# jl6017/AutoURDF

Measured on AMD Instinct MI355X. Metric: registered frames/sec (N=4096 pts, K=20 clusters), higher is better.
Workload: dtype f32

## Files before the change

autourdf_amd/csrc/train_engine.hip:

```cpp
#include <cfloat>
#include <chrono>
#include <cmath>
#include <cstdlib>
#include <cstring>
#include <type_traits>
#include <vector>
#include "creg_common.h"
#include "nn_l1.h"

namespace creg {

struct Dims {
    int rot, K, KP, IN, H, HA, HB, H2, OA, OB, NP, NT, epochs;
    float slope;
    int oW1, ob1, oW2, ob2, oW3A, ob3A, oW3B, ob3B, NPAR;
    int nbx, nby;
    int nyb;
    int npb;
    int ppl;
    int nbt, nbp;
    int rows;
};

constexpr int PS_MAXB = 512;
// ... 535 lines not shown
                const unsigned idx = (unsigned)(key[sl] & 0xFFFFull);
                unsigned u = 0xFFFFFFFFu;
                if (idx != 0xFFFFu) {
                    const float4 p = W.pts4[idx];
                    u = ordered_bits(axis == 0 ? p.x : axis == 1 ? p.y : p.z);
                }
                key[sl] = ((unsigned long long)u << 16) | idx;
            }
            __syncthreads();
            bitonic_segments(key, npow, 64 >> sub, tid, 512);
        }
    for (int sl = tid; sl < ns; sl += 512) {
        const unsigned idx = (unsigned)(key[sl] & 0xFFFFull);
        float4 o = make_float4(0.f, 0.f, 0.f, __int_as_float(0x7fffffff));
        if (idx != 0xFFFFu) { const float4 p = W.pts4[idx]; o = make_float4(p.x, p.y, p.z, __int_as_float((int)idx)); }
        W.psl4[(size_t)first * BS + sl] = o;
    }
}

struct EngineEpi {
    int* sgn_x; int4* cnt4; float* lossp_x; float* lossp_y;
    size_t bstride;
    const int* stopped;
    __device__ __forceinline__ void shift(int z) {
        const size_t b = (size_t)z * bstride;
        sgn_x = (int*)((char*)sgn_x + b); cnt4 = (int4*)((char*)cnt4 + b);
        lossp_x = (float*)((char*)lossp_x + b); lossp_y = (float*)((char*)lossp_y + b);
        stopped = (const int*)((const char*)stopped + b);
    }
    __device__ __forceinline__ void operator()(int dir, int q, int idx, float d, float qx, float qy, float qz,
                                               float tx, float ty, float tz, float& acc) const {
        if (dir == 0) {
            sgn_x[q] = (qx > tx ? 1 : 0) | (qy > ty ? 2 : 0) | (qz > tz ? 4 : 0);
        } else {
            atomicAdd(&cnt4[idx].x, (qx > tx) ? -1 : 1);
            atomicAdd(&cnt4[idx].y, (qy > ty) ? -1 : 1);
            atomicAdd(&cnt4[idx].z, (qz > tz) ? -1 : 1);
        }
        acc += d;
    }
    __device__ __forceinline__ void finish(int dir, int blk, float s, float*) const { (dir == 0 ? lossp_x : lossp_y)[blk] = s; }
};

template <bool P1, int PPL, int NBT, int NBP>
__global__ __launch_bounds__(NN_BLOCK) void k_nn_plan(const float* A, int na, const float* B, int nb, int blocksA,
                                                      int blocksB, EngineEpi epi, NnBlocks yb, NnBlocks pb, size_t zstride) {
    asm volatile("" :: "s"(A), "s"(na), "s"(B), "s"(nb), "s"(blocksA), "s"(blocksB), "s"(epi.sgn_x), "s"(epi.cnt4), "s"(epi.lossp_x), "s"(epi.lossp_y),
                 "s"(epi.bstride), "s"(epi.stopped), "s"(yb.ts4), "s"(yb.tbox), "s"(yb.nblk), "s"(pb.ts4), "s"(pb.tbox), "s"(pb.nblk_dev), "s"(zstride));
    const int nz = gridDim.x / (blocksA + blocksB);
    int i = blockIdx.x, z, bx;
    if (i < blocksB * nz) { z = i / blocksB; bx = blocksA + (i - z * blocksB); }
    else { i -= blocksB * nz; z = i / blocksA; bx = i - z * blocksA; }
    const size_t zb = z * zstride;
    A = (const float*)((const char*)A + zb);
    B = (const float*)((const char*)B + zb);
    yb.ts4 = (const float4*)((const char*)yb.ts4 + zb);
    yb.tbox = (const float*)((const char*)yb.tbox + zb);
    epi.shift(z);
    if (bx < blocksA) nn_l1_block_pruned<NBT, PPL, EngineEpi, true, false>(A, na, 4, yb, 0, epi, bx, epi.stopped, B, 4);
    else if constexpr (P1) {
        pb.ts4 = (const float4*)((const char*)pb.ts4 + zb);
        pb.tbox = (const float*)((const char*)pb.tbox + zb);
        pb.nblk_dev = (const int*)((const char*)pb.nblk_dev + zb);
        nn_l1_block_pruned<NBP, PPL, EngineEpi, true, true>(B, nb, 4, pb, 1, epi, bx - blocksA, epi.stopped, A, 4);
    } else nn_l1_block<4, int, EngineEpi>(A, na, 4, B, nb, 4, nullptr, nullptr, nullptr, nullptr, blocksA, epi, bx);
}

template <int NBT, int NBP>
__global__ __launch_bounds__(NN_ROWS_BLOCK) void k_nn_rows(const float* A, const float* B, int blocksA, int blocksB, EngineEpi epi, NnBlocks yb, NnBlocks pb,
                                                      size_t zstride) {
    asm volatile("" :: "s"(A), "s"(B), "s"(blocksA), "s"(blocksB), "s"(epi.sgn_x), "s"(epi.cnt4), "s"(epi.lossp_x), "s"(epi.lossp_y),
                 "s"(epi.bstride), "s"(epi.stopped), "s"(yb.ts4), "s"(yb.tbox), "s"(yb.nblk), "s"(pb.ts4), "s"(pb.tbox), "s"(pb.nblk_dev), "s"(zstride));
    const int nz = gridDim.x / (blocksA + blocksB);
    int i = blockIdx.x, z, bx;
    if (i < blocksB * nz) { z = i / blocksB; bx = blocksA + (i - z * blocksB); }
    else { i -= blocksB * nz; z = i / blocksA; bx = i - z * blocksA; }
    const size_t zb = z * zstride;
    A = (const float*)((const char*)A + zb);
    B = (const float*)((const char*)B + zb);
    yb.ts4 = (const float4*)((const char*)yb.ts4 + zb);
    yb.tbox = (const float*)((const char*)yb.tbox + zb);
    pb.ts4 = (const float4*)((const char*)pb.ts4 + zb);
    pb.tbox = (const float*)((const char*)pb.tbox + zb);
    pb.nblk_dev = (const int*)((const char*)pb.nblk_dev + zb);
    epi.shift(z);
    if (bx < blocksA) nn_l1_rows<NBT, EngineEpi, false, true>(pb.ts4, 0, pb.nblk_dev, pb.nblk, yb, 0, epi, bx, epi.stopped, B, epi.lossp_x);
    else nn_l1_rows<NBP, EngineEpi, true, false>(yb.ts4, yb.nblk, nullptr, yb.nblk, pb, 1, epi, bx - blocksA, epi.stopped, A, epi.lossp_y);
}

__device__ __forceinline__ TrainState advance_state(const TrainState& S, float loss, const Hyper& hy, double bc1, float bc2_sqrt) {
    TrainState N = S;
    const bool improved = loss < S.min_loss;
    N.last_loss = loss;
    N.epochs_run = S.epochs_run + 1;
    const int count = improved ? 0 : S.count + 1;
    N.min_loss = improved ? loss : S.min_loss;
    N.best_epoch = improved ? S.epochs_run : S.best_epoch;
    N.count = count;
    N.stopped = (!improved && count > hy.stop) ? 1 : S.stopped;
    if (!N.stopped) {
        N.step = S.step + 1;
        N.step_size = (float)(S.lr / bc1);
        N.bc2_sqrt = bc2_sqrt;
        const double cur = (double)loss;
        if (cur < S.sched_best * (1.0 - 1e-4)) { N.sched_best = cur; N.sched_bad = 0; }
        else N.sched_bad = S.sched_bad + 1;
        if (N.sched_bad > hy.patience) {
            const double nl = fmax(S.lr * (double)hy.factor, 0.0);
            if (S.lr - nl > 1e-8) N.lr = nl;
            N.sched_bad = 0;
        }
    }
    return N;
}

constexpr int GC_QMAX = 3;
__device__ __forceinline__ void gradc_role(const Dims& D, const Ws& W, int epoch, int nbx, int nby, int k) {
    __shared__ float red[4][14];
    __shared__ float s_loss;
    __shared__ float s_go[16];
    const int tid = threadIdx.x, lane = tid & 63, wv = tid >> 6;
    const TrainState S = W.state[epoch & 1];
    const int b0 = W.off[k], e0 = W.off[k + 1];
    const Hyper hy = *W.hyper;
    float a = tid < nbx ? W.lossp_x[tid] : 0.f, b = tid < nby ? W.lossp_y[tid] : 0.f;
    const float m2v = W.m2[16 * k + (tid & 15)];
    float sv[16];
#pragma unroll
    for (int i = 0; i < 16; ++i) sv[i] = W.head_save[16 * k + i];
    const float* h2cur = (epoch & 1) ? W.h2[1] : W.h2[0];
    float w3v[GC_QMAX][8], h2v[GC_QMAX];
#pragma unroll
    for (int q = 0; q < GC_QMAX; ++q) {
        const int o = min(q * 256 + tid, D.H2 - 1);
        const bool isA = o < D.HA;
        const float* Pc = (epoch & 1) ? W.P1 : W.P;
        const float* wb = isA ? Pc + D.oW3A + o : Pc + D.oW3B + (o - D.HA);
        const int stride = isA ? D.HA : D.HB, nj = isA ? D.OA : D.OB;
#pragma unroll
        for (int j = 0; j < 8; ++j) w3v[q][j] = wb[(size_t)min(j, nj - 1) * stride];
        h2v[q] = h2cur[(size_t)k * D.H2 + o];
    }
    asm volatile("" :: "v"(a), "v"(b), "v"(m2v), "v"(sv[0]), "v"(sv[1]), "v"(sv[2]), "v"(sv[3]), "v"(sv[4]), "v"(sv[5]), "v"(sv[6]), "v"(sv[7]),
                 "v"(sv[8]), "v"(sv[9]), "v"(sv[10]), "v"(sv[11]), "v"(sv[12]), "v"(sv[13]), "v"(sv[14]), "v"(sv[15]), "v"(b0), "v"(e0), "v"(hy.lr));
#pragma unroll
    for (int q = 0; q < GC_QMAX; ++q)
        asm volatile("" :: "v"(h2v[q]), "v"(w3v[q][0]), "v"(w3v[q][1]), "v"(w3v[q][2]), "v"(w3v[q][3]), "v"(w3v[q][4]), "v"(w3v[q][5]), "v"(w3v[q][6]),
                     "v"(w3v[q][7]));
    if (S.stopped) {
        if (k == 0 && tid == 0) {
            TrainState E = S; E.stopped = 1;
            W.state[(epoch + 1) & 1] = E;
        }
        return;
    }
    const int n_first = min(b0 + tid, D.NP - 1);
    const float4 p_first = W.pts4[n_first];
    const int4 c_first = W.cnt4[n_first];
    const int s_first = W.sgn_x[n_first];
    const float4 pr_first = W.pred4[n_first];
    for (int i = tid + 256; i < nbx; i += 256) a += W.lossp_x[i];
    for (int i = tid + 256; i < nby; i += 256) b += W.lossp_y[i];
    a = wave_sum_fast(a); b = wave_sum_fast(b);
    if (lane == 0) { red[wv][0] = a; red[wv][1] = b; }
    __syncthreads();
    if (tid == 0) {
        const float sa = ((red[0][0] + red[1][0]) + red[2][0]) + red[3][0];
        const float sb = ((red[0][1] + red[1][1]) + red[2][1]) + red[3][1];
        s_loss = sa / (float)D.NP + sb / (float)D.NT;
    }
    __syncthreads();
    const float loss = s_loss;
    TrainState N = advance_state(S, loss, hy, S.next_bc1, S.next_bc2s);
    const bool improved = loss < S.min_loss;
    if (improved) {
        for (int n = b0 + tid; n < e0; n += 256) {
            const float4 p = (n == b0 + tid) ? pr_first : W.pred4[n];
            W.best_pred[3 * (size_t)n] = p.x; W.best_pred[3 * (size_t)n + 1] = p.y; W.best_pred[3 * (size_t)n + 2] = p.z;
        }
        if (tid < 16) W.best_m[16 * k + tid] = m2v;
    }
    if (k == 0 && tid == 0) {
        N.next_bc1 = W.bc1[min(N.step + 1, D.epochs)];
        N.next_bc2s = W.bc2s[min(N.step + 1, D.epochs)];
        W.state[(epoch + 1) & 1] = N;
        W.loss_hist[S.epochs_run] = loss;
        W.lr_hist[S.epochs_run] = (float)S.lr;
        W.result[0] = N.min_loss; W.result[1] = (float)N.epochs_run; W.result[2] = (float)N.lr; W.result[3] = (float)N.best_epoch;
    }
    if (N.stopped) return;
    const float gx = 1.0f / (float)D.NP, gy = 1.0f / (float)D.NT;
    float acc[12];
#pragma unroll
    for (int i = 0; i < 12; ++i) acc[i] = 0.f;
    for (int n = b0 + tid; n < e0; n += 256) {
        const bool first = n == b0 + tid;
        const float4 p = first ? p_first : W.pts4[n];
        const int4 c = first ? c_first : W.cnt4[n];
        const int sb = first ? s_first : W.sgn_x[n];
        const float g[3] = {((sb & 1) ? gx : -gx) + gy * (float)c.x, ((sb & 2) ? gx : -gx) + gy * (float)c.y,
                            ((sb & 4) ? gx : -gx) + gy * (float)c.z};
#pragma unroll
        for (int q = 0; q < 3; ++q) {
            acc[4 * q] = fmaf(g[q], p.x, acc[4 * q]); acc[4 * q + 1] = fmaf(g[q], p.y, acc[4 * q + 1]);
            acc[4 * q + 2] = fmaf(g[q], p.z, acc[4 * q + 2]); acc[4 * q + 3] += g[q];
        }
    }
    __syncthreads();
#pragma unroll
    for (int i = 0; i < 12; ++i) { const float r = wave_sum_fast(acc[i]); if (lane == 0) red[wv][i] = r; }
    __syncthreads();
    if (tid == 0) {
        float G12[12];
        for (int i = 0; i < 12; ++i) G12[i] = ((red[0][i] + red[1][i]) + red[2][i]) + red[3][i];
        for (int i = 0; i < 16; ++i) W.gm2[16 * k + i] = i < 12 ? G12[i] : 0.f;
        const float G[9] = {G12[0], G12[1], G12[2], G12[4], G12[5], G12[6], G12[8], G12[9], G12[10]};
        const float gt[3] = {G12[3], G12[7], G12[11]};
        float go[16];
        for (int i = 0; i < 16; ++i) go[i] = 0.f;
        if (D.rot == ROT_6D) {
            go[0] = gt[0]; go[1] = gt[1]; go[2] = gt[2];
            rot6d_to_matrix_vjp(sv, G, go + 4);
        } else if (D.rot == ROT_RPY) {
            go[0] = gt[0]; go[1] = gt[1]; go[2] = gt[2];
            float ge[3];
            euler_xyz_to_matrix_vjp(sv, G, ge);
            for (int i = 0; i < 3; ++i) go[4 + i] = ge[i] * (1.f - sv[4 + i] * sv[4 + i]);
        } else if (D.rot == ROT_Q) {
            go[0] = gt[0]; go[1] = gt[1]; go[2] = gt[2];
            float gu[4];
            quat_to_matrix_vjp(sv, G, gu);
            const float nrm = sv[4];
            if (nrm > 1e-12f) {
                const float dot = sv[0] * gu[0] + sv[1] * gu[1] + sv[2] * gu[2] + sv[3] * gu[3];
#pragma unroll
                for (int i = 0; i < 4; ++i) go[4 + i] = (gu[i] - sv[i] * dot) / nrm;
            } else {
#pragma unroll
                for (int i = 0; i < 4; ++i) go[4 + i] = gu[i] / 1e-12f;
            }
        } else {
            float gdq[8];
            dq_to_se3_vjp(sv, G, gt, gdq);
            for (int i = 0; i < 8; ++i) go[4 + i] = gdq[i];
        }
        for (int i = 0; i < 12; ++i) { W.g_out[16 * k + i] = go[i]; s_go[i] = go[i]; }
    }
    __syncthreads();
#pragma unroll
    for (int q = 0; q < GC_QMAX; ++q) {
        const int o = q * 256 + tid;
        if (o < D.H2) {
            const bool isA = o < D.HA;
            const int nj = isA ? D.OA : D.OB, gofs = isA ? 0 : 4;
            float sum = 0.f;
#pragma unroll
            for (int j = 0; j < 8; ++j) if (j < nj) sum = fmaf(s_go[gofs + j], w3v[q][j], sum);
            W.g_h2[(size_t)k * D.H2 + o] = sum * act_grad(h2v[q], D.slope);
        }
    }
}

__global__ __launch_bounds__(256) void k_gradc(Dims D, Ws W0, int epoch, int nbx, int nby, size_t bstride) {
    asm volatile("" :: "s"(W0.P), "s"(W0.P1), "s"(W0.h2[0]), "s"(W0.h2[1]), "s"(W0.head_save), "s"(W0.m2), "s"(W0.gm2), "s"(W0.pts4), "s"(W0.pred4),
                 "s"(W0.sgn_x), "s"(W0.cnt4), "s"(W0.lossp_x), "s"(W0.lossp_y), "s"(W0.g_out), "s"(W0.g_h2), "s"(W0.state), "s"(W0.bc1), "s"(W0.bc2s),
                 "s"(W0.best_m), "s"(W0.best_pred), "s"(W0.loss_hist), "s"(W0.lr_hist), "s"(W0.result), "s"(W0.off), "s"(W0.hyper),
                 "s"(D.rot), "s"(D.K), "s"(D.H2), "s"(D.HA), "s"(D.HB), "s"(D.OA), "s"(D.OB), "s"(D.NP), "s"(D.NT), "s"(D.epochs), "s"(D.slope),
                 "s"(D.oW3A), "s"(D.oW3B), "s"(epoch), "s"(nbx), "s"(nby), "s"(bstride));
    const Ws W = ws_shift(W0, blockIdx.z * bstride);
    gradc_role(D, W, epoch, nbx, nby, blockIdx.x);
}

__device__ __forceinline__ float adam_value(float p, float& mm, float& vv, float g, float step_size, float bc2_sqrt) {
    const float b1w = (float)(1.0 - 0.9), b2 = 0.999f, b2w = (float)(1.0 - 0.999);
    mm = mm + b1w * (g - mm);
    vv = vv * b2 + (b2w * g) * g;
    const float denom = sqrtf(vv) / bc2_sqrt + 1e-8f;
    return p + (-step_size * mm) / denom;
}

#ifdef CREG_BD_STAMPS
struct BdStamps {
    unsigned long long first[256], endB[256], endD[256], startB[256], startD[256];
    unsigned long long phase[2][8], blocks[2];
    int armed;
};
__device__ BdStamps g_bd_st;
#define BD_T0 unsigned long long bd_t[8]; int bd_n = 0; if (threadIdx.x == 0) bd_t[bd_n++] = bd_entry;
#define BD_T  if (threadIdx.x == 0) bd_t[bd_n++] = wall_clock64();
#define BD_TEND(role, epoch) do { asm volatile("s_waitcnt vmcnt(0)" ::: "memory"); if (threadIdx.x == 0) { bd_t[bd_n++] = wall_clock64(); \
    if (g_bd_st.armed) { const int sl_ = (epoch) & 255; atomicMin(&g_bd_st.first[sl_], bd_t[0]); \
        atomicMin(role ? &g_bd_st.startD[sl_] : &g_bd_st.startB[sl_], bd_t[0]); atomicMax(role ? &g_bd_st.endD[sl_] : &g_bd_st.endB[sl_], bd_t[bd_n - 1]); \
        for (int k_ = 1; k_ < bd_n; ++k_) atomicAdd(&g_bd_st.phase[role][k_ - 1], bd_t[k_] - bd_t[k_ - 1]); atomicAdd(&g_bd_st.blocks[role], 1ull); } } } while (0)
#else
#define BD_T0
#define BD_T
#define BD_TEND(role, epoch)
#endif
constexpr int BD_THREADS = 512;
constexpr int B2_THREADS = BD_THREADS;
constexpr int B2_WAVES = B2_THREADS / 64;
constexpr int B2_CB = 16;
constexpr int B2_RB = 32;
__host__ __device__ inline int b2_smem_floats(int K, int IN, int H2) {
    return B2_WAVES * B2_RB * B2_CB + K * IN + 2 * K * B2_CB + H2 * B2_CB;
}
__device__ __forceinline__ float row_sum16(float v) {
    CREG_DPP_STEP(v, 0xB1, 0xF);
    CREG_DPP_STEP(v, 0x4E, 0xF);
    CREG_DPP_STEP(v, 0x141, 0xF);
    CREG_DPP_STEP(v, 0x140, 0xF);
    return v;
}

template <int KW, bool X>
__device__ __forceinline__ void bwd2_role(const Dims& D, const Ws& W, int epoch, int blk, float* sh, unsigned long long bd_entry) {
    constexpr int NS = KW / 4;
    constexpr bool V4 = KW % 16 == 0;
    constexpr int NA = V4 ? NS / 4 : NS;
    float* red = sh;
    float* encs = red + B2_WAVES * B2_RB * B2_CB;
    float* gxs = encs + D.K * D.IN;
    float* xt = gxs + D.K * B2_CB;
    float* w2s = xt + D.K * B2_CB;
    const int tid = threadIdx.x, lane = tid & 63, wv = tid >> 6, lj = lane & 15, kk = lane >> 4;
    __builtin_amdgcn_s_waitcnt(0x0F70);
    const int c0 = blk * B2_CB, par = epoch & 1;
    const float* x1cur = par ? W.x1[1] : W.x1[0];
    float* x1next = par ? W.x1[0] : W.x1[1];
    const float* Pc = par ? W.P1 : W.P;
    float* Pn = par ? W.P : W.P1;
    BD_T0
    {
        const float* src = Pc + D.oW2 + (size_t)(wv * KW + (lane >> 2)) * D.H + c0 + 4 * (lane & 3);
        float* dst = w2s + wv * KW * B2_CB;
#pragma unroll
        for (int i = 0; i < KW; i += 16)
            if (i + (lane >> 2) < KW)
                __builtin_amdgcn_global_load_lds((const __attribute__((address_space(1))) void*)(src + (size_t)i * D.H),
                                                 (__attribute__((address_space(3))) void*)(dst + i * B2_CB), 16, 0, 0);
    }
    const float* gbase = W.g_h2 + wv * KW + (V4 ? 4 * kk : kk);
    auto load_a = [&](int row, float* dst) {
        const float* g = gbase + (size_t)min(row, D.K - 1) * D.H2;
#pragma unroll
        for (int q = 0; q < NA; ++q) {
            if constexpr (V4) { const float4 v = *(const float4*)(g + 16 * q); dst[4 * q] = v.x; dst[4 * q + 1] = v.y; dst[4 * q + 2] = v.z; dst[4 * q + 3] = v.w; }
            else dst[q] = g[4 * q];
        }
    };
    float a0[NS], a1[NS];
    const bool two0 = D.K > 16;
    load_a(lj, a0);
    if (two0) load_a(16 + lj, a1);
    const int half = tid >> 8, t2 = tid & 255, row = t2 >> 4, i4 = t2 & 15, hu = c0 + row;
    const bool ain = 4 * i4 < D.IN;
    const int ei = min(4 * i4, D.IN - 4);
    const size_t wi = (size_t)D.oW1 + (size_t)hu * D.IN + ei;
    float4 pw = *(const float4*)(Pc + wi), pm = *(const float4*)(W.AM + wi), pv = *(const float4*)(W.AV + wi);
    const bool ain2 = X && 64 + 4 * i4 < D.IN;
    const int ei2 = min(64 + 4 * i4, D.IN - 4);
    const size_t wi2 = (size_t)D.oW1 + (size_t)hu * D.IN + ei2;
    float4 pw2, pm2, pv2;
    if constexpr (X) { pw2 = *(const float4*)(Pc + wi2); pm2 = *(const float4*)(W.AM + wi2); pv2 = *(const float4*)(W.AV + wi2); }
    float pb = Pc[D.ob1 + hu], mb = W.AM[D.ob1 + hu], vb = W.AV[D.ob1 + hu];
    float xv0 = x1cur[(size_t)min(tid >> 4, D.K - 1) * D.H + c0 + (tid & 15)];
    {
        const int n = D.K * D.IN / 4;
        constexpr int NPC = 8;
#pragma unroll
        for (int c = 0; c < NPC; ++c) {
            const int i = c * B2_THREADS + tid;
            if (i < n)
                __builtin_amdgcn_global_load_lds((const __attribute__((address_space(1))) void*)((const float4*)W.enc + i),
                                                 (__attribute__((address_space(3))) void*)((float4*)encs + c * B2_THREADS + (tid & ~63)), 16, 0, 0);
        }
    }
    __builtin_amdgcn_sched_barrier(0);
    const TrainState S = W.state[(epoch + 1) & 1];
    const bool live = !S.stopped;
    __builtin_amdgcn_sched_barrier(0);
    BD_T
    stage_wait();
    float wb[NS];
#pragma unroll
    for (int s = 0; s < NS; ++s) {
        const int o = V4 ? 16 * (s >> 2) + 4 * kk + (s & 3) : 4 * s + kk;
        wb[s] = w2s[(wv * KW + o) * B2_CB + lj];
    }
    for (int r0 = 0; r0 < D.K; r0 += B2_RB) {
        const int nr = min(B2_RB, D.K - r0);
        const bool two = nr > 16;
        float xv = xv0;
        if (r0) {
            load_a(r0 + lj, a0);
            if (two) load_a(r0 + 16 + lj, a1);
            xv = x1cur[(size_t)min(r0 + (tid >> 4), D.K - 1) * D.H + c0 + (tid & 15)];
        }
        f32x4 acc0 = {0.f, 0.f, 0.f, 0.f}, acc1 = {0.f, 0.f, 0.f, 0.f};
        if (two) {
#pragma unroll
            for (int s = 0; s < NS; ++s) {
                acc0 = __builtin_amdgcn_mfma_f32_16x16x4f32(a0[s], wb[s], acc0, 0, 0, 0);
                acc1 = __builtin_amdgcn_mfma_f32_16x16x4f32(a1[s], wb[s], acc1, 0, 0, 0);
            }
        } else {
#pragma unroll
            for (int s = 0; s < NS; ++s) acc0 = __builtin_amdgcn_mfma_f32_16x16x4f32(a0[s], wb[s], acc0, 0, 0, 0);
        }
        if (r0) __syncthreads();
        {
            float* o = red + (wv * B2_RB + 4 * kk) * B2_CB + lj;
#pragma unroll
            for (int v = 0; v < 4; ++v) { o[v * B2_CB] = acc0[v]; if (two) o[(16 + v) * B2_CB] = acc1[v]; }
        }
        stage_wait();
        __syncthreads();
        if (r0 == 0) { BD_T }
        if (!live) return;
        if (tid < nr * B2_CB) {
            float sum = red[tid];
#pragma unroll
            for (int w2 = 1; w2 < B2_WAVES; ++w2) sum += red[w2 * B2_RB * B2_CB + tid];
            gxs[r0 * B2_CB + tid] = sum * act_grad(xv, D.slope);
        }
    }
    __syncthreads();
    BD_T
    float4 ag = make_float4(0.f, 0.f, 0.f, 0.f), ag2 = make_float4(0.f, 0.f, 0.f, 0.f);
    float gsum = 0.f;
    for (int r = 0; r < D.K; ++r) {
        const float g = gxs[r * B2_CB + row];
        const float4 e = *(const float4*)(encs + r * D.IN + ei);
        ag.x = fmaf(g, e.x, ag.x); ag.y = fmaf(g, e.y, ag.y); ag.z = fmaf(g, e.z, ag.z); ag.w = fmaf(g, e.w, ag.w);
        if constexpr (X) {
            const float4 e2 = *(const float4*)(encs + r * D.IN + ei2);
            ag2.x = fmaf(g, e2.x, ag2.x); ag2.y = fmaf(g, e2.y, ag2.y); ag2.z = fmaf(g, e2.z, ag2.z); ag2.w = fmaf(g, e2.w, ag2.w);
        }
        gsum += g;
    }
    float4 nw;
    nw.x = adam_value(pw.x, pm.x, pv.x, ag.x, S.step_size, S.bc2_sqrt);
    nw.y = adam_value(pw.y, pm.y, pv.y, ag.y, S.step_size, S.bc2_sqrt);
    nw.z = adam_value(pw.z, pm.z, pv.z, ag.z, S.step_size, S.bc2_sqrt);
    nw.w = adam_value(pw.w, pm.w, pv.w, ag.w, S.step_size, S.bc2_sqrt);
    float4 nw2 = make_float4(0.f, 0.f, 0.f, 0.f);
    if constexpr (X) {
        nw2.x = adam_value(pw2.x, pm2.x, pv2.x, ag2.x, S.step_size, S.bc2_sqrt);
        nw2.y = adam_value(pw2.y, pm2.y, pv2.y, ag2.y, S.step_size, S.bc2_sqrt);
        nw2.z = adam_value(pw2.z, pm2.z, pv2.z, ag2.z, S.step_size, S.bc2_sqrt);
        nw2.w = adam_value(pw2.w, pm2.w, pv2.w, ag2.w, S.step_size, S.bc2_sqrt);
    }
    pb = adam_value(pb, mb, vb, gsum, S.step_size, S.bc2_sqrt);
    if (live && half == 0) {
        if (ain) { st4_wt(Pn, wi, nw); st4_wt(W.AM, wi, pm); st4_wt(W.AV, wi, pv); }
        if constexpr (X) if (ain2) { st4_wt(Pn, wi2, nw2); st4_wt(W.AM, wi2, pm2); st4_wt(W.AV, wi2, pv2); }
        if (i4 == 0) { Pn[D.ob1 + hu] = pb; W.AM[D.ob1 + hu] = mb; W.AV[D.ob1 + hu] = vb; }
    }
    BD_T
    for (int r = half; r < D.K; r += 2) {
        const float4 e = *(const float4*)(encs + r * D.IN + ei);
        float v = ain ? fmaf(nw.w, e.w, fmaf(nw.z, e.z, fmaf(nw.y, e.y, nw.x * e.x))) : 0.f;
        if constexpr (X) {
            const float4 e2 = *(const float4*)(encs + r * D.IN + ei2);
            if (ain2) v = fmaf(nw2.w, e2.w, fmaf(nw2.z, e2.z, fmaf(nw2.y, e2.y, fmaf(nw2.x, e2.x, v))));
        }
        v = row_sum16(v) + pb;
        if (i4 == 0) xt[r * B2_CB + row] = act_f(v, D.slope);
    }
    __syncthreads();
    if (live)
        for (int t = tid; t < D.K * (B2_CB / 2); t += B2_THREADS) {
            const int r = t >> 3, c2 = 2 * (t & 7);
            *(nn_f2*)(x1next + (size_t)r * D.H + c0 + c2) = nn_f2{xt[r * B2_CB + c2], xt[r * B2_CB + c2 + 1]};
        }
    BD_TEND(0, epoch);
}


constexpr int DW_UNITS = 16;
constexpr int DW_TILES = 4;
constexpr int DW_KC = 5;
__host__ __device__ inline int dw_blocks(const Dims& D) { return D.H2 / DW_UNITS + 2; }

__device__ __forceinline__ void dw_role(const Dims& D, const Ws& W, int epoch, int blk, unsigned long long bd_entry) {
    const int lane = threadIdx.x & 63, wv = threadIdx.x >> 6, lj = lane & 15, q = lane >> 4;
    __builtin_amdgcn_s_waitcnt(0x0F70);
    const int par = epoch & 1;
    const float* Pc = par ? W.P1 : W.P;
    float* Pn = par ? W.P : W.P1;
    const float* x1cur = par ? W.x1[1] : W.x1[0];
    const float* h2cur = par ? W.h2[1] : W.h2[0];
    asm volatile("" : "+s"(x1cur), "+s"(h2cur));
    const int nb2 = D.H2 / DW_UNITS;
    int u0, nu, n_in, oW, ob, astride, gstride;
    const float *amat, *gmat;
    if (blk < nb2) { u0 = blk * DW_UNITS; nu = DW_UNITS; n_in = D.H; oW = D.oW2 + u0 * D.H; ob = D.ob2 + u0; amat = x1cur; astride = D.H; gmat = W.g_h2 + u0; gstride = D.H2; }
    else if (blk == nb2) { u0 = 0; nu = D.OA; n_in = D.HA; oW = D.oW3A; ob = D.ob3A; amat = h2cur; astride = D.H2; gmat = W.g_out; gstride = 16; }
    else { u0 = 0; nu = D.OB; n_in = D.HB; oW = D.oW3B; ob = D.ob3B; amat = h2cur + D.HA; astride = D.H2; gmat = W.g_out + 4; gstride = 16; }
    if (nu == 0) return;
    if (64 * wv >= n_in) return;
    BD_T0
    const int unit = min(lj, nu - 1);
    const bool ulive = lj < nu;
    const int i0 = 64 * wv;
    const int po = (oW + unit * n_in + i0 + 4 * q) * 4;
    const __amdgpu_buffer_rsrc_t rP = buf_rsrc(Pc, D.NPAR * 4), rM = buf_rsrc(W.AM, D.NPAR * 4), rV = buf_rsrc(W.AV, D.NPAR * 4);
    f32x4 acc[DW_TILES];
#pragma unroll
    for (int t = 0; t < DW_TILES; ++t) acc[t] = f32x4{0.f, 0.f, 0.f, 0.f};
    float gb = 0.f;
    const __amdgpu_buffer_rsrc_t rA = buf_rsrc(amat, (D.KP * astride - (int)(amat - (blk < nb2 ? x1cur : h2cur))) * 4);
    const __amdgpu_buffer_rsrc_t rG = buf_rsrc(gmat, (D.KP * gstride - (blk < nb2 ? u0 : (blk == nb2 ? 0 : 4))) * 4);
    const int aoff = (q * astride + i0 + 16 * (lj & 3) + 4 * (lj >> 2)) * 4, goff = (q * gstride + unit) * 4;
    float bop[DW_KC];
    float4 aop[DW_KC];
    auto load_ops = [&](int s0) {
#pragma unroll
        for (int s = 0; s < DW_KC; ++s) {
            const int r4 = 4 * (s0 + s);
            bop[s] = __uint_as_float(__builtin_amdgcn_raw_buffer_load_b32(rG, goff, r4 * gstride * 4, 0));
            aop[s] = ld_buf4(rA, aoff, r4 * astride * 4);
        }
    };
    auto mfma_ops = [&]() {
#pragma unroll
        for (int s = 0; s < DW_KC; ++s) {
            acc[0] = __builtin_amdgcn_mfma_f32_16x16x4f32(aop[s].x, bop[s], acc[0], 0, 0, 0);
            acc[1] = __builtin_amdgcn_mfma_f32_16x16x4f32(aop[s].y, bop[s], acc[1], 0, 0, 0);
            acc[2] = __builtin_amdgcn_mfma_f32_16x16x4f32(aop[s].z, bop[s], acc[2], 0, 0, 0);
            acc[3] = __builtin_amdgcn_mfma_f32_16x16x4f32(aop[s].w, bop[s], acc[3], 0, 0, 0);
        }
#pragma unroll
        for (int s = 0; s < DW_KC; ++s) gb += bop[s];
    };
    load_ops(0);
    __builtin_amdgcn_sched_barrier(0);
    const TrainState S = W.state[(epoch + 1) & 1];
    float pb = Pc[ob + unit], mb = W.AM[ob + unit], vb = W.AV[ob + unit];
    __builtin_amdgcn_sched_barrier(0);
    float4 pw[DW_TILES], pm[DW_TILES], pv[DW_TILES];
    bool vl[DW_TILES];
#pragma unroll
    for (int v = 0; v < DW_TILES; ++v) {
        vl[v] = ulive && i0 + 16 * v + 4 * q < n_in;
        pw[v] = ld_buf4(rP, po + 64 * v, 0); pm[v] = ld_buf4(rM, po + 64 * v, 0); pv[v] = ld_buf4(rV, po + 64 * v, 0);
        __builtin_amdgcn_sched_barrier(0);
    }
    BD_T
    mfma_ops();
    for (int s0 = DW_KC; 4 * s0 < D.KP; s0 += DW_KC) {
        load_ops(s0);
        __builtin_amdgcn_sched_barrier(0);
        mfma_ops();
    }
    BD_T
    if (S.stopped) return;
#pragma unroll
    for (int v = 0; v < DW_TILES; ++v) {
        float4 nw;
        nw.x = adam_value(pw[v].x, pm[v].x, pv[v].x, acc[0][v], S.step_size, S.bc2_sqrt);
        nw.y = adam_value(pw[v].y, pm[v].y, pv[v].y, acc[1][v], S.step_size, S.bc2_sqrt);
        nw.z = adam_value(pw[v].z, pm[v].z, pv[v].z, acc[2][v], S.step_size, S.bc2_sqrt);
        nw.w = adam_value(pw[v].w, pm[v].w, pv[v].w, acc[3][v], S.step_size, S.bc2_sqrt);
        if (vl[v]) { const int e = po / 4 + 16 * v; st4_wt(Pn, e, nw); st4_wt(W.AM, e, pm[v]); st4_wt(W.AV, e, pv[v]); }
    }
    if (wv == 0) {
        float sum = gb;
        sum += __shfl_xor(gb, 16, 64);
        sum += __shfl_xor(sum, 32, 64);
        pb = adam_value(pb, mb, vb, sum, S.step_size, S.bc2_sqrt);
        if (q == 0 && ulive) { Pn[ob + unit] = pb; W.AM[ob + unit] = mb; W.AV[ob + unit] = vb; }
    }
    BD_TEND(1, epoch);
}

template <int NC, int KW, bool X = false>
__global__ __launch_bounds__(BD_THREADS, 4) void k_bd(Dims D, Ws W0, int epoch, size_t bstride, int nz) {
    extern __shared__ __attribute__((aligned(16))) char smem[];
#ifdef CREG_BD_STAMPS
    const unsigned long long bd_entry = wall_clock64();
#else
    const unsigned long long bd_entry = 0;
#endif
#ifndef CREG_BD_NO_TOUCH
    asm volatile("" :: "s"(W0.P), "s"(W0.P1), "s"(W0.AM), "s"(W0.AV), "s"(W0.enc), "s"(W0.x1[0]), "s"(W0.x1[1]), "s"(W0.h2[0]), "s"(W0.h2[1]),
                 "s"(W0.g_out), "s"(W0.g_h2), "s"(W0.state), "s"(D.K), "s"(D.KP), "s"(D.IN), "s"(D.H), "s"(D.H2), "s"(D.HA), "s"(D.HB), "s"(D.OA),
                 "s"(D.OB), "s"(D.oW1), "s"(D.ob1), "s"(D.oW2), "s"(D.ob2), "s"(D.oW3A), "s"(D.ob3A), "s"(D.oW3B), "s"(D.ob3B), "s"(D.NPAR),
                 "s"(D.slope), "s"(epoch), "s"(bstride), "s"(nz));
#endif
    const int nB = D.H / B2_CB, nD = dw_blocks(D);
    int i = blockIdx.x;
    const bool roleB = i < nB * nz;
    if (!roleB) i -= nB * nz;
    const int n = roleB ? nB : nD, z = i / n, blk = i - z * n;
    const Ws W = ws_shift(W0, (size_t)z * bstride);
#ifdef CREG_BD_ONLY
    if ((CREG_BD_ONLY == 1) != roleB) return;
#endif
    if (roleB) bwd2_role<KW, X>(D, W, epoch, blk, (float*)smem, bd_entry);
    else dw_role(D, W, epoch, blk, bd_entry);
}

__global__ __launch_bounds__(256) void k_params_home(Dims D, Ws W0, size_t bstride, int sidx, int step0) {
    const Ws W = ws_shift(W0, blockIdx.z * bstride);
    if (((W.state[sidx].step - step0) & 1) == 0) return;
    for (int i = blockIdx.x * 256 + threadIdx.x; i < D.NPAR; i += gridDim.x * 256) W.P[i] = W.P1[i];
}

struct ResumeState { double lr, sched_best; int step, epochs_run, sched_bad, count, best_epoch, stopped; float min_loss; };
__global__ void k_set_state(Dims D, Ws W, ResumeState rs) {
    if (threadIdx.x || blockIdx.x) return;
    TrainState s = W.state[0];
    s.lr = rs.lr; s.sched_best = rs.sched_best; s.sched_bad = rs.sched_bad; s.count = rs.count; s.stopped = rs.stopped; s.step = rs.step;
    s.min_loss = rs.min_loss; s.epochs_run = rs.epochs_run; s.best_epoch = rs.best_epoch;
    s.next_bc1 = W.bc1[min(rs.step + 1, D.epochs)]; s.next_bc2s = W.bc2s[min(rs.step + 1, D.epochs)];
    W.state[0] = s; W.state[1] = s;
    W.result[0] = s.min_loss; W.result[1] = (float)s.epochs_run; W.result[2] = (float)s.lr; W.result[3] = (float)s.best_epoch;
}
__global__ void k_get_state(Ws W, int sidx, double* out) {
    if (threadIdx.x || blockIdx.x) return;
    const TrainState s = W.state[sidx];
    out[0] = s.step; out[1] = s.epochs_run; out[2] = s.lr; out[3] = s.sched_best; out[4] = s.sched_bad; out[5] = s.count;
    out[6] = (double)s.min_loss; out[7] = s.best_epoch; out[8] = s.stopped; out[9] = (double)s.last_loss; out[10] = 0.0; out[11] = 0.0;
}

struct Plan {
    creg_train_shape shape;
    Dims D;
    Ws W;
    char* base;
    size_t bytes;
    hipGraphExec_t gexec;
    bool graph_ready;
    int graph_epochs;
    int B;
    int nz;
    size_t bstride;
    int smem_bd;
    int branches;
    bool chain_streams;
    hipStream_t cst[8];
    hipGraphExec_t cexec[8];
    hipEvent_t cfork, cjoin[8];
    hipStream_t cal_stream;
    bool cal_done;
    int probe_us;
    bool target_blocks_valid;
};

static bool make_dims(const creg_train_shape* s, Dims* D) {
    if (!s || s->rot < 0 || s->rot > 3 || s->k < 1 || s->k > 256 || (s->hidden != 64 && s->hidden != 128 && s->hidden != 256 && s->hidden != 512) || s->epochs < 1 || s->n_pred < 1 || s->n_tgt < 1 || s->n_pred >= (1ll << 31) ||
        s->n_tgt >= (1ll << 31))
        return false;
    memset(D, 0, sizeof(*D));
    D->rot = s->rot; D->K = s->k; D->KP = (s->k + 19) / 20 * 20; D->H = s->hidden; D->NP = (int)s->n_pred; D->NT = (int)s->n_tgt; D->epochs = s->epochs;
    if (s->rot == ROT_Q) { D->IN = 56; D->HA = D->H / 2; D->HB = D->H; D->OA = 3; D->OB = 4; D->slope = 0.01f; }
    else if (s->rot == ROT_DQ) { D->IN = 64; D->HA = 0; D->HB = D->H; D->OA = 0; D->OB = 8; D->slope = 0.f; }
    else if (s->rot == ROT_6D) { D->IN = 72; D->HA = D->H / 2; D->HB = D->H; D->OA = 3; D->OB = 6; D->slope = 0.01f; }
    else { D->IN = 48; D->HA = D->H / 2; D->HB = D->H; D->OA = 3; D->OB = 3; D->slope = 0.01f; }
    if (D->K * D->IN / 4 > 8 * 512) return false;
    D->H2 = D->HA + D->HB;
    if (sizeof(float) * b2_smem_floats(D->K, D->IN, D->H2) > 160 * 1024) return false;
    int o = 0;
    D->oW1 = o; o += D->H * D->IN; D->ob1 = o; o += D->H;
    D->oW2 = o; o += D->H2 * D->H; D->ob2 = o; o += D->H2;
    D->oW3A = o; o += D->OA * D->HA; D->ob3A = o; o += D->OA;
    D->oW3B = o; o += D->OB * D->HB; D->ob3B = o; o += D->OB;
    D->NPAR = o;
    if (D->H2 % 32 || D->H % B2_CB || D->H2 > 256 * GC_QMAX) return false;
    const NnGrid g = nn_grid(D->NP, D->NT, true, true, 4);
    D->nbx = g.blocksA; D->nby = g.blocksB;
    const bool rows_fit = D->NT <= 16384 && D->NP < 65535 && (D->NP + 63) / 64 + D->K <= PS_MAXB && g.qw == 4;
    const char* rows_env = getenv("CREG_NN_ROWS");
    const bool rows_pays = D->NT > 64 * 64;
    D->rows = s->nn_search == 0 && rows_fit && (rows_env ? rows_env[0] == '1' : rows_pays);
    D->ppl = (D->rows || D->NT <= 64 * 64) ? 1 : 4;
    const int BS = 64 * D->ppl;
    D->nyb = (s->nn_search != 1 && D->NT <= 4 * YS_CHUNK && g.qw == 4) ? (D->NT + BS - 1) / BS : 0;
    D->npb = (D->nyb && D->NP < 65535 && (D->NP + BS - 1) / BS + D->K <= PS_MAXB) ? (D->NP + BS - 1) / BS + D->K : 0;
    const int nt = (D->nyb + 63) / 64, np = (D->npb + 63) / 64;
    D->nbt = nt <= 1 ? 1 : (nt <= 2 ? 2 : 4);
    D->nbp = np <= 2 ? 2 : (np <= 3 ? 3 : (np <= 4 ? 4 : (np <= 5 ? 5 : (np <= 6 ? 6 : 8))));
    if (D->rows) { D->nbx = 4 * D->npb; D->nby = 4 * D->nyb; }
    return true;
}

static size_t carve(const Dims& D, char* base, Ws* W) {
    size_t o = 0;
    auto take = [&](size_t bytes) -> char* { char* r = base ? base + o : nullptr; o = align_up(o + bytes, 256); return r; };
    const size_t f = sizeof(float);
    Ws w;
    w.P = (float*)take(f * D.NPAR); w.P1 = (float*)take(f * D.NPAR); w.AM = (float*)take(f * D.NPAR); w.AV = (float*)take(f * D.NPAR);
    w.pose_in = (float*)take(f * POSE_IN * D.K); w.enc = (float*)take(f * D.K * D.IN);
    w.x1[0] = (float*)take(f * D.KP * D.H); w.x1[1] = (float*)take(f * D.KP * D.H);
    w.h2[0] = (float*)take(f * D.KP * D.H2); w.h2[1] = (float*)take(f * D.KP * D.H2); w.head_save = (float*)take(f * 16 * D.K);
    w.m2 = (float*)take(f * 16 * D.K); w.gm2 = (float*)take(f * 16 * D.K);
    w.pts4 = (float4*)take(sizeof(float4) * D.NP); w.y4 = (float4*)take(sizeof(float4) * D.NT);
    w.pred4 = (float4*)take(sizeof(float4) * D.NP);
    const size_t bs = 64 * (size_t)D.ppl;
    w.ys4 = (float4*)take(sizeof(float4) * bs * (D.nyb ? D.nyb : 1)); w.ybox = (float*)take(f * 6 * 64 * D.nbt);
    w.psl4 = (float4*)take(sizeof(float4) * bs * (D.npb ? D.npb : 1)); w.ps4 = (float4*)take(sizeof(float4) * bs * (D.npb ? D.npb : 1));
    w.pbox = (float*)take(f * 6 * 64 * D.nbp); w.sb = (int*)take(sizeof(int) * (D.K + 1));
    w.sgn_x = (int*)take(sizeof(int) * D.NP);
    w.cnt4 = (int4*)take(sizeof(int4) * D.NP);
    w.lossp_x = (float*)take(f * D.nbx); w.lossp_y = (float*)take(f * D.nby);
    w.g_out = (float*)take(f * 16 * D.KP); w.g_h2 = (float*)take(f * D.KP * D.H2);
    w.state = (TrainState*)take(sizeof(TrainState) * 2);
    w.bc1 = (double*)take(sizeof(double) * (D.epochs + 1)); w.bc2s = (float*)take(f * (D.epochs + 1));
    w.best_m = (float*)take(f * 16 * D.K); w.best_pred = (float*)take(f * 3 * D.NP);
    w.loss_hist = (float*)take(f * D.epochs); w.lr_hist = (float*)take(f * D.epochs); w.result = (float*)take(f * 4);
    w.off = (int*)take(sizeof(int) * (D.K + 1)); w.hyper = (Hyper*)take(sizeof(Hyper));
    w.ysum = (unsigned long long*)take(sizeof(unsigned long long) * 4);
    if (W) *W = w;
    return o;
}

template <typename F>
static void by_nc(int H, F f) {
    switch (H / 64) {
        case 1: f(std::integral_constant<int, 1>{}); break;
        case 2: f(std::integral_constant<int, 2>{}); break;
        case 4: f(std::integral_constant<int, 4>{}); break;
        default: f(std::integral_constant<int, 8>{}); break;
    }
}
static void launch_l2(Plan* P, int par, hipStream_t s) {
    const Dims& D = P->D; const Ws& W = P->W;
    by_nc(D.H, [&](auto nc) {
        hipLaunchKernelGGL((k_l2<decltype(nc)::value>), dim3(D.H2 / 16, 1, P->nz), dim3(L2_THREADS), 0, s, D, W, par, P->bstride); });
}
static void launch_head(Plan* P, int par, hipStream_t s) {
    const Dims& D = P->D; const Ws& W = P->W;
    by_nc(D.H, [&](auto nc) {
        if (D.OA + D.OB > 8) hipLaunchKernelGGL((k_head<decltype(nc)::value, true>), dim3(D.K, 1, P->nz), dim3(512), 0, s, D, W, par, P->bstride);
        else hipLaunchKernelGGL((k_head<decltype(nc)::value>), dim3(D.K, 1, P->nz), dim3(512), 0, s, D, W, par, P->bstride);
    });
}
template <typename F>
static void by_bd(const Dims& D, F f) {
    by_nc(D.H, [&](auto nc) {
        constexpr int NC = decltype(nc)::value;
        if (D.IN > 64) f(k_bd<NC, 12 * NC, true>);
        else if (D.HA) f(k_bd<NC, 12 * NC>);
        else f(k_bd<NC, 8 * NC>);
    });
}
static void launch_bd(Plan* P, int epoch, hipStream_t s) {
    const Dims& D = P->D; const Ws& W = P->W;
    const int per = D.H / B2_CB + dw_blocks(D);
    by_bd(D, [&](auto kern) { hipLaunchKernelGGL(kern, dim3(per * P->nz), dim3(BD_THREADS), P->smem_bd, s, D, W, epoch, P->bstride, P->nz); });
}
static void launch_nn(const Dims& D, const Ws& W, size_t bstride, int nz, hipStream_t s, int par = 0) {
    const EngineEpi epi{W.sgn_x, W.cnt4, W.lossp_x, W.lossp_y, bstride, &W.state[par].stopped};
    if (D.rows) {
        const NnBlocks yb{W.ys4, W.ybox, D.nyb, nullptr}, pb{W.ps4, W.pbox, D.npb, W.sb + D.K};
        const int blocksA = cdiv(64 * D.npb, NN_ROW_SLOTS), blocksB = cdiv(64 * D.nyb, NN_ROW_SLOTS);
        const dim3 grid((blocksA + blocksB) * nz);
        auto go = [&](auto kern) {
            hipLaunchKernelGGL(kern, grid, dim3(NN_ROWS_BLOCK), 0, s, (const float*)W.pred4, (const float*)W.y4, blocksA, blocksB, epi, yb, pb, bstride);
        };
        auto pick_p = [&](auto nbt) {
            constexpr int NBT = decltype(nbt)::value;
            switch (D.nbp) {
                case 2: go(k_nn_rows<NBT, 2>); break;
                case 3: go(k_nn_rows<NBT, 3>); break;
                case 4: go(k_nn_rows<NBT, 4>); break;
                case 5: go(k_nn_rows<NBT, 5>); break;
                case 6: go(k_nn_rows<NBT, 6>); break;
                default: go(k_nn_rows<NBT, 8>); break;
            }
        };
        switch (D.nbt) {
            case 1: pick_p(std::integral_constant<int, 1>{}); break;
            case 2: pick_p(std::integral_constant<int, 2>{}); break;
            default: pick_p(std::integral_constant<int, 4>{}); break;
        }
    } else if (D.nyb) {
// ... 651 lines not shown
```

Baseline: 164.8.

## Split W1 Adam update to one half-block and batch forward row reductions

```diff
diff --git a/autourdf_amd/csrc/train_engine.hip b/autourdf_amd/csrc/train_engine.hip
--- a/autourdf_amd/csrc/train_engine.hip
+++ b/autourdf_amd/csrc/train_engine.hip
@@ -861,8 +861,9 @@
 constexpr int B2_WAVES = B2_THREADS / 64;
 constexpr int B2_CB = 16;
 constexpr int B2_RB = 32;
+constexpr int B2_NR = 5;
 __host__ __device__ inline int b2_smem_floats(int K, int IN, int H2) {
-    return B2_WAVES * B2_RB * B2_CB + K * IN + 2 * K * B2_CB + H2 * B2_CB;
+    return B2_WAVES * B2_RB * B2_CB + K * IN + K * B2_CB + H2 * B2_CB;
 }
 __device__ __forceinline__ float row_sum16(float v) {
     CREG_DPP_STEP(v, 0xB1, 0xF);
@@ -880,8 +881,7 @@
     float* red = sh;
     float* encs = red + B2_WAVES * B2_RB * B2_CB;
     float* gxs = encs + D.K * D.IN;
-    float* xt = gxs + D.K * B2_CB;
-    float* w2s = xt + D.K * B2_CB;
+    float* w2s = gxs + D.K * B2_CB;
     const int tid = threadIdx.x, lane = tid & 63, wv = tid >> 6, lj = lane & 15, kk = lane >> 4;
     __builtin_amdgcn_s_waitcnt(0x0F70);
     const int c0 = blk * B2_CB, par = epoch & 1;
@@ -916,13 +916,19 @@
     const bool ain = 4 * i4 < D.IN;
     const int ei = min(4 * i4, D.IN - 4);
     const size_t wi = (size_t)D.oW1 + (size_t)hu * D.IN + ei;
-    float4 pw = *(const float4*)(Pc + wi), pm = *(const float4*)(W.AM + wi), pv = *(const float4*)(W.AV + wi);
+    const float4 f4z = make_float4(0.f, 0.f, 0.f, 0.f);
+    float4 pw = f4z, pm = f4z, pv = f4z, pw2 = f4z, pm2 = f4z, pv2 = f4z;
+    float pb = 0.f, mb = 0.f, vb = 0.f;
+    if (half == 0) {
+        pw = *(const float4*)(Pc + wi); pm = *(const float4*)(W.AM + wi); pv = *(const float4*)(W.AV + wi);
+    }
     const bool ain2 = X && 64 + 4 * i4 < D.IN;
     const int ei2 = min(64 + 4 * i4, D.IN - 4);
     const size_t wi2 = (size_t)D.oW1 + (size_t)hu * D.IN + ei2;
-    float4 pw2, pm2, pv2;
-    if constexpr (X) { pw2 = *(const float4*)(Pc + wi2); pm2 = *(const float4*)(W.AM + wi2); pv2 = *(const float4*)(W.AV + wi2); }
-    float pb = Pc[D.ob1 + hu], mb = W.AM[D.ob1 + hu], vb = W.AV[D.ob1 + hu];
+    if (half == 0) {
+        if constexpr (X) { pw2 = *(const float4*)(Pc + wi2); pm2 = *(const float4*)(W.AM + wi2); pv2 = *(const float4*)(W.AV + wi2); }
+        pb = Pc[D.ob1 + hu]; mb = W.AM[D.ob1 + hu]; vb = W.AV[D.ob1 + hu];
+    }
     float xv0 = x1cur[(size_t)min(tid >> 4, D.K - 1) * D.H + c0 + (tid & 15)];
     {
         const int n = D.K * D.IN / 4;
@@ -986,53 +992,77 @@
     }
     __syncthreads();
     BD_T
-    float4 ag = make_float4(0.f, 0.f, 0.f, 0.f), ag2 = make_float4(0.f, 0.f, 0.f, 0.f);
-    float gsum = 0.f;
-    for (int r = 0; r < D.K; ++r) {
-        const float g = gxs[r * B2_CB + row];
-        const float4 e = *(const float4*)(encs + r * D.IN + ei);
-        ag.x = fmaf(g, e.x, ag.x); ag.y = fmaf(g, e.y, ag.y); ag.z = fmaf(g, e.z, ag.z); ag.w = fmaf(g, e.w, ag.w);
+    float4 nw = f4z, nw2 = f4z;
+    float4* hw = (float4*)red;
+    if (half == 0) {
+        float4 ag = f4z, ag2 = f4z;
+        float gsum = 0.f;
+        for (int r = 0; r < D.K; ++r) {
+            const float g = gxs[r * B2_CB + row];
+            const float4 e = *(const float4*)(encs + r * D.IN + ei);
+            ag.x = fmaf(g, e.x, ag.x); ag.y = fmaf(g, e.y, ag.y); ag.z = fmaf(g, e.z, ag.z); ag.w = fmaf(g, e.w, ag.w);
+            if constexpr (X) {
+                const float4 e2 = *(const float4*)(encs + r * D.IN + ei2);
+                ag2.x = fmaf(g, e2.x, ag2.x); ag2.y = fmaf(g, e2.y, ag2.y); ag2.z = fmaf(g, e2.z, ag2.z); ag2.w = fmaf(g, e2.w, ag2.w);
+            }
+            gsum += g;
+        }
+        nw.x = adam_value(pw.x, pm.x, pv.x, ag.x, S.step_size, S.bc2_sqrt);
+        nw.y = adam_value(pw.y, pm.y, pv.y, ag.y, S.step_size, S.bc2_sqrt);
+        nw.z = adam_value(pw.z, pm.z, pv.z, ag.z, S.step_size, S.bc2_sqrt);
+        nw.w = adam_value(pw.w, pm.w, pv.w, ag.w, S.step_size, S.bc2_sqrt);
         if constexpr (X) {
-            const float4 e2 = *(const float4*)(encs + r * D.IN + ei2);
-            ag2.x = fmaf(g, e2.x, ag2.x); ag2.y = fmaf(g, e2.y, ag2.y); ag2.z = fmaf(g, e2.z, ag2.z); ag2.w = fmaf(g, e2.w, ag2.w);
-        }
-        gsum += g;
-    }
-    float4 nw;
-    nw.x = adam_value(pw.x, pm.x, pv.x, ag.x, S.step_size, S.bc2_sqrt);
-    nw.y = adam_value(pw.y, pm.y, pv.y, ag.y, S.step_size, S.bc2_sqrt);
-    nw.z = adam_value(pw.z, pm.z, pv.z, ag.z, S.step_size, S.bc2_sqrt);
-    nw.w = adam_value(pw.w, pm.w, pv.w, ag.w, S.step_size, S.bc2_sqrt);
-    float4 nw2 = make_float4(0.f, 0.f, 0.f, 0.f);
-    if constexpr (X) {
-        nw2.x = adam_value(pw2.x, pm2.x, pv2.x, ag2.x, S.step_size, S.bc2_sqrt);
-        nw2.y = adam_value(pw2.y, pm2.y, pv2.y, ag2.y, S.step_size, S.bc2_sqrt);
-        nw2.z = adam_value(pw2.z, pm2.z, pv2.z, ag2.z, S.step_size, S.bc2_sqrt);
-        nw2.w = adam_value(pw2.w, pm2.w, pv2.w, ag2.w, S.step_size, S.bc2_sqrt);
-    }
-    pb = adam_value(pb, mb, vb, gsum, S.step_size, S.bc2_sqrt);
-    if (live && half == 0) {
-        if (ain) { st4_wt(Pn, wi, nw); st4_wt(W.AM, wi, pm); st4_wt(W.AV, wi, pv); }
-        if constexpr (X) if (ain2) { st4_wt(Pn, wi2, nw2); st4_wt(W.AM, wi2, pm2); st4_wt(W.AV, wi2, pv2); }
-        if (i4 == 0) { Pn[D.ob1 + hu] = pb; W.AM[D.ob1 + hu] = mb; W.AV[D.ob1 + hu] = vb; }
+            nw2.x = adam_value(pw2.x, pm2.x, pv2.x, ag2.x, S.step_size, S.bc2_sqrt);
+            nw2.y = adam_value(pw2.y, pm2.y, pv2.y, ag2.y, S.step_size, S.bc2_sqrt);
+            nw2.z = adam_value(pw2.z, pm2.z, pv2.z, ag2.z, S.step_size, S.bc2_sqrt);
+            nw2.w = adam_value(pw2.w, pm2.w, pv2.w, ag2.w, S.step_size, S.bc2_sqrt);
+        }
+        pb = adam_value(pb, mb, vb, gsum, S.step_size, S.bc2_sqrt);
+        if (live) {
+            if (ain) { st4_wt(Pn, wi, nw); st4_wt(W.AM, wi, pm); st4_wt(W.AV, wi, pv); }
+            if constexpr (X) if (ain2) { st4_wt(Pn, wi2, nw2); st4_wt(W.AM, wi2, pm2); st4_wt(W.AV, wi2, pv2); }
+            if (i4 == 0) { Pn[D.ob1 + hu] = pb; W.AM[D.ob1 + hu] = mb; W.AV[D.ob1 + hu] = vb; }
+        }
+        hw[t2] = nw;
+        if constexpr (X) hw[256 + t2] = nw2;
+        if (i4 == 0) red[2048 + row] = pb;
     }
     BD_T
-    for (int r = half; r < D.K; r += 2) {
-        const float4 e = *(const float4*)(encs + r * D.IN + ei);
-        float v = ain ? fmaf(nw.w, e.w, fmaf(nw.z, e.z, fmaf(nw.y, e.y, nw.x * e.x))) : 0.f;
-        if constexpr (X) {
-            const float4 e2 = *(const float4*)(encs + r * D.IN + ei2);
-            if (ain2) v = fmaf(nw2.w, e2.w, fmaf(nw2.z, e2.z, fmaf(nw2.y, e2.y, fmaf(nw2.x, e2.x, v))));
-        }
-        v = row_sum16(v) + pb;
-        if (i4 == 0) xt[r * B2_CB + row] = act_f(v, D.slope);
-    }
     __syncthreads();
-    if (live)
-        for (int t = tid; t < D.K * (B2_CB / 2); t += B2_THREADS) {
-            const int r = t >> 3, c2 = 2 * (t & 7);
-            *(nn_f2*)(x1next + (size_t)r * D.H + c0 + c2) = nn_f2{xt[r * B2_CB + c2], xt[r * B2_CB + c2 + 1]};
-        }
+    if (half) {
+        nw = hw[t2];
+        if constexpr (X) nw2 = hw[256 + t2];
+        pb = red[2048 + row];
+    }
+    for (int rb = half; rb < D.K; rb += 2 * B2_NR) {
+        float4 e[B2_NR], e2[B2_NR];
+#pragma unroll
+        for (int j = 0; j < B2_NR; ++j) {
+            const int r = min(rb + 2 * j, D.K - 1);
+            e[j] = *(const float4*)(encs + r * D.IN + ei);
+            if constexpr (X) e2[j] = *(const float4*)(encs + r * D.IN + ei2);
+        }
+        float v[B2_NR];
+#pragma unroll
+        for (int j = 0; j < B2_NR; ++j) {
+            v[j] = ain ? fmaf(nw.w, e[j].w, fmaf(nw.z, e[j].z, fmaf(nw.y, e[j].y, nw.x * e[j].x))) : 0.f;
+            if constexpr (X)
+                if (ain2) v[j] = fmaf(nw2.w, e2[j].w, fmaf(nw2.z, e2[j].z, fmaf(nw2.y, e2[j].y, fmaf(nw2.x, e2[j].x, v[j]))));
+        }
+#pragma unroll
+        for (int j = 0; j < B2_NR; ++j) CREG_DPP_STEP(v[j], 0xB1, 0xF);
+#pragma unroll
+        for (int j = 0; j < B2_NR; ++j) CREG_DPP_STEP(v[j], 0x4E, 0xF);
+#pragma unroll
+        for (int j = 0; j < B2_NR; ++j) CREG_DPP_STEP(v[j], 0x141, 0xF);
+#pragma unroll
+        for (int j = 0; j < B2_NR; ++j) CREG_DPP_STEP(v[j], 0x140, 0xF);
+        float out = act_f(v[0] + pb, D.slope);
+#pragma unroll
+        for (int j = 1; j < B2_NR; ++j) { const float a = act_f(v[j] + pb, D.slope); out = i4 == j ? a : out; }
+        const int r = rb + 2 * i4;
+        if (live && i4 < B2_NR && r < D.K) x1next[(size_t)r * D.H + c0 + row] = out;
+    }
     BD_TEND(0, epoch);
 }
 
```

After: 167.2 (median of 6 runs). +1.5%, better.
